# hsinnan75/Dart

Hardware: AMD Instinct MI355X
Metric: M paired-end reads/sec (2x101 bp vs GRCh38-sized index), host to host; records bit-identical to CPU dart (higher is better)
Workload: dtype u64/u8 integer

## Files before the change

### dart_amd/csrc/dg_api.hip

```cpp
#include "../../include/dartgpu.h"
#include "dg_common.h"
#include "dg_fm.h"
#include "dg_seedq.h"
#include "dg_chain.h"
#include "dg_report.h"
#include "dg_pair.h"
#include "dg_reseed.h"
#include "dg_sort.h"
#include "dg_samfmt.h"
#include "dg_bamfmt.h"
#include "dg_bgzf.h"
#include "dg_bgzf_dyn.h"
#include "dg_fastq.h"
#include "dg_inflate.h"
#include "dg_sjtab.h"
#include "dg_bamsort.h"
#include "dg_bamidx.h"
#include "dg_coverage.h"
#include "dg_markdup.h"
#include "dg_pileup.h"
#include "dg_qc.h"
#include "dg_tags.h"
#include "dg_genecount.h"
#include "dg_rnametrics.h"
#include <stdio.h>
#include <stdlib.h>
#include <string.h>
#include <string>
#include <algorithm>
#include <vector>
#include <atomic>
#include <mutex>
#include <chrono>
#include <thread>
#include <condition_variable>
#include <fcntl.h>
#include <unistd.h>
#include <sys/stat.h>

static char g_init_error[512] = "";

#define DG_HW_QUEUES_NEED 16
static_assert(DG_HW_QUEUES_NEED <= 32, "more hardware queues than 32 are not asked for");
static char g_hwq_found[24] = "unset";
static int g_hwq_left = DG_HW_QUEUES_NEED;
__attribute__((constructor)) static void dg_default_hw_queues()
{
    const char *v = getenv("GPU_MAX_HW_QUEUES");
    long have = 0;
    if (v) {
        size_t i = 0;
        for (; v[i] && i + 1 < sizeof g_hwq_found; i++) g_hwq_found[i] = (v[i] > ' ' && v[i] < 127 && v[i] != ';' && v[i] != '=') ? v[i] : '?';
        g_hwq_found[i] = 0;
        if (!i) snprintf(g_hwq_found, sizeof g_hwq_found, "empty");
        char *end = nullptr;
        have = strtol(v, &end, 10);
        if (end == v || *end) have = 0; else if (have > 1000000) have = 1000000;
    }
    if (have < DG_HW_QUEUES_NEED) {
// ... 786 lines not shown
    if (!parent) return nullptr;
    hipError_t e;
    if ((e = hipSetDevice(parent->device)) != hipSuccess) { if (status) *status = DG_ERR_HIP; return nullptr; }
    dg_ctx *c = new dg_ctx();
    c->device = parent->device; c->owns_index = false; c->n_cu = parent->n_cu;
    c->shared_ix = parent->shared_ix;
    c->ix = parent->ix; c->ix_gen = parent->ix_gen; c->pr = parent->pr;
    refresh_index(c);
    c->shared_caps = parent->shared_caps;
    if ((e = make_ctx_objects(c)) != hipSuccess) {
        snprintf(g_init_error, sizeof g_init_error, "dg_clone: %s", hipGetErrorString(e)); dg_destroy(c); if (status) *status = DG_ERR_HIP; return nullptr;
    }
    const int live = g_live_ctx[c->device & 63].load();
    if (live + 2 > g_hwq_left && !g_hwq_warned.exchange(true))
        fprintf(stderr, "[libdartgpu] %d contexts on device %d + the copy stream + the caller's stream are more than the %d hardware queues of this process "
                        "(GPU_MAX_HW_QUEUES was %s when the library loaded and %d when its constructor returned): contexts will share queues and wait for each other\n",
                live, c->device, g_hwq_left, g_hwq_found, g_hwq_left);
    if (status) *status = DG_OK;
    return c;
}

static int enqueue_upload(dg_ctx *c, int n_reads, const uint32_t *seq_off, const uint16_t *rlen, const char *seq)
{
    if (!c || n_reads < 0 || (n_reads > 0 && (!seq_off || !rlen || !seq))) return DG_ERR_ARG;
    HIPCHK(hipSetDevice(c->device));
    size_t bytes = 0; int mx = 0;
    for (int i = 0; i < n_reads; i++) {
        const size_t end = (size_t)seq_off[i] + rlen[i];
        bytes = end > bytes ? end : bytes;
        mx = rlen[i] > mx ? rlen[i] : mx;
    }
    if (mx > DG_MAX_RLEN) { snprintf(c->err, 512, "a read is longer than DG_MAX_RLEN (%d)", DG_MAX_RLEN); return DG_ERR_ARG; }
    c->n_reads = n_reads; c->max_rlen = mx; c->seq_bytes = bytes; c->enc_ready = false; c->enqueued = false; c->batch_done = false; c->sj.batch_counted = false; c->gc.batch_counted = false; c->sam.valid = false; c->bam.valid = false; c->bam.rec_valid = false; c->bam.rec_stored = false; c->fq.valid = false;
    c->no_batch = false; c->inf.valid = false;
    HIPCHK(c->seq.ensure(bytes + 64));
    HIPCHK(c->seq_off.ensure((size_t)n_reads + 1)); HIPCHK(c->rlen.ensure((size_t)n_reads + 1));
    if (n_reads) {
        HIPCHK(hipMemcpyAsync(c->seq.p, seq, bytes, hipMemcpyHostToDevice, c->stream));
        HIPCHK(hipMemcpyAsync(c->seq_off.p, seq_off, (size_t)n_reads * 4, hipMemcpyHostToDevice, c->stream));
        HIPCHK(hipMemcpyAsync(c->rlen.p, rlen, (size_t)n_reads * 2, hipMemcpyHostToDevice, c->stream));
    }
    return DG_OK;
}

extern "C" int dg_batch_upload(dg_ctx *c, int n_reads, const uint32_t *seq_off, const uint16_t *rlen, const char *seq)
{
    const int rc = enqueue_upload(c, n_reads, seq_off, rlen, seq);
    if (rc) return rc;
    HIPCHK(hipStreamSynchronize(c->stream));
    return DG_OK;
}

__global__ void __launch_bounds__(256)
k_unpack(const uint32_t *__restrict__ words, uint32_t n_words, int W2, double inv_w2, int rlen_all, const uint16_t *rlen_in, unsigned char *__restrict__ seq,
         uint32_t *__restrict__ seq_off, uint16_t *rlen_out, uint32_t *__restrict__ enc, unsigned int *bad)
{
    const uint32_t t = blockIdx.x * blockDim.x + threadIdx.x;
    if (t >= n_words) return;
    if (t == 0) *bad = 0u;
    uint32_t r = (uint32_t)((double)t * inv_w2);
    if (r * (uint32_t)W2 > t) r--; else if ((r + 1u) * (uint32_t)W2 <= t) r++;
    const int ww = (int)(t - r * (uint32_t)W2);
    const int len = rlen_in ? rlen_in[r] : rlen_all, left = len - 16 * ww;
    const uint32_t w = words[t];
    const uint32_t past = left >= 16 ? 0u : (left <= 0 ? 0xFFFFFFFFu : 0xFFFFFFFFu >> (2 * left));
    enc[(size_t)r * 2 * W2 + ww] = w & ~past;
    enc[(size_t)r * 2 * W2 + W2 + ww] = past;
    if (ww == 0) { seq_off[r] = r * 16u * (uint32_t)W2; if (!rlen_in) rlen_out[r] = (uint16_t)len; }
}
__global__ void __launch_bounds__(256)
k_unpack_n(const uint32_t *__restrict__ nlist, uint32_t n_n, int W2, uint32_t n_bases, unsigned char *__restrict__ seq, uint32_t *__restrict__ enc, unsigned int *bad)
{
    const uint32_t i = blockIdx.x * blockDim.x + threadIdx.x;
    if (i >= n_n) return;
    const uint32_t flat = nlist[i], per = 16u * (uint32_t)W2, r = flat / per, pos = flat - r * per;
    if (flat >= n_bases) { atomicMax(bad, 1u); return; }
    const uint32_t bit = 3u << (30 - 2 * (pos & 15u));
    atomicAnd(&enc[(size_t)r * 2 * W2 + (pos >> 4)], ~bit);
    atomicOr(&enc[(size_t)r * 2 * W2 + W2 + (pos >> 4)], bit);
}

static int enqueue_upload_packed(dg_ctx *c, int n_reads, int rlen_all, const uint16_t *rlen, int words_per_read, const uint32_t *words, const uint32_t *nlist, size_t n_n)
{
    if (!c || n_reads < 0 || words_per_read < 1 || (n_reads > 0 && !words) || (n_n > 0 && !nlist)) return DG_ERR_ARG;
    HIPCHK(hipSetDevice(c->device));
    const int W2 = words_per_read;
    int mx = rlen_all;
    if (rlen) { mx = 0; for (int i = 0; i < n_reads; i++) mx = rlen[i] > mx ? rlen[i] : mx; }
    if (mx > DG_MAX_RLEN || mx > 16 * W2 || (size_t)n_reads * 16 * W2 > 0xFFFFFFF0ull) { snprintf(c->err, 512, "packed batch: read length %d does not fit %d words (or exceeds DG_MAX_RLEN / 2^32 bases)", mx, W2); return DG_ERR_ARG; }
    if (n_reads && (mx + 15) / 16 != W2) { snprintf(c->err, 512, "packed batch: words_per_read must be ceil(longest read / 16) = %d", (mx + 15) / 16); return DG_ERR_ARG; }
    const size_t nw = (size_t)n_reads * W2, bytes = nw * 16;
    c->n_reads = n_reads; c->max_rlen = mx; c->seq_bytes = bytes; c->enqueued = false; c->batch_done = false; c->sj.batch_counted = false; c->gc.batch_counted = false; c->sam.valid = false; c->bam.valid = false; c->bam.rec_valid = false; c->bam.rec_stored = false; c->fq.valid = false;
    c->no_batch = false; c->inf.valid = false;
    HIPCHK(c->seq.ensure(bytes + 64)); HIPCHK(c->seq_off.ensure((size_t)n_reads + 1)); HIPCHK(c->rlen.ensure((size_t)n_reads + 1));
    HIPCHK(c->enc.ensure(2 * nw + 16)); HIPCHK(c->packed_in.ensure(nw + 1)); HIPCHK(c->nlist_in.ensure(n_n + 1));
    c->enc_ready = true;
    if (n_reads == 0) return DG_OK;
    HIPCHK(hipMemcpyAsync(c->packed_in.p, words, nw * 4, hipMemcpyHostToDevice, c->stream));
    if (rlen) HIPCHK(hipMemcpyAsync(c->rlen.p, rlen, (size_t)n_reads * 2, hipMemcpyHostToDevice, c->stream));
    if (n_n) HIPCHK(hipMemcpyAsync(c->nlist_in.p, nlist, n_n * 4, hipMemcpyHostToDevice, c->stream));
    k_unpack<<<(unsigned)((nw + 255) / 256), 256, 0, c->stream>>>(c->packed_in.p, (uint32_t)nw, W2, 1.0 / (double)W2, rlen_all, rlen ? c->rlen.p : nullptr, c->seq.p, c->seq_off.p, c->rlen.p, c->enc.p, c->d_input_bad);
    if (n_n) {
        k_unpack_n<<<(unsigned)((n_n + 255) / 256), 256, 0, c->stream>>>(c->nlist_in.p, (uint32_t)n_n, W2, (uint32_t)(nw * 16), c->seq.p, c->enc.p, c->d_input_bad);
        HIPCHK(hipMemcpyAsync(&c->h_tail->input_bad, c->d_input_bad, 4, hipMemcpyDeviceToHost, c->stream));
    } else c->h_tail->input_bad = 0;
    HIPCHK(hipGetLastError());
    return DG_OK;
}

extern "C" int dg_batch_upload_packed(dg_ctx *c, int n_reads, int rlen_all, const uint16_t *rlen, int words_per_read, const uint32_t *words, const uint32_t *nlist, size_t n_n)
{
    const int rc = enqueue_upload_packed(c, n_reads, rlen_all, rlen, words_per_read, words, nlist, n_n);
    if (rc) return rc;
    HIPCHK(hipStreamSynchronize(c->stream));
    return DG_OK;
}

extern "C" int dg_fastq_tile(void) { return FQ_TILE; }

struct FqPlan { size_t n[2], off2, line_cap[2], tile_stride, reads_bound, len_tiles, max_reads, text_bytes; bool two; };

static int fq_reserve(dg_ctx *c, FqPlan &p)
{
    HIPCHK(c->fq.ready());
    const size_t max_reads = p.max_reads, n1 = p.n[0], n2 = p.n[1];
    const size_t rec_cap[2] = { p.two ? (max_reads + 1) / 2 : max_reads, p.two ? max_reads / 2 : 0 };
    size_t tiles[2];
    for (int f = 0; f < 2; f++) { p.line_cap[f] = std::min(4 * rec_cap[f] + 1, p.n[f] + 1); tiles[f] = (p.n[f] + FQ_TILE - 1) / FQ_TILE; }
    p.off2 = (n1 + 16 + 255) & ~(size_t)255; p.text_bytes = n1 + n2;
    p.tile_stride = std::max(tiles[0], tiles[1]);
    p.reads_bound = std::min(max_reads, (n1 + 4) / 4 + (n2 + 4) / 4);
    p.len_tiles = std::max<size_t>(1, (p.reads_bound + FQ_THREADS - 1) / FQ_THREADS);
    const size_t reads_bound = p.reads_bound, text_bytes = p.text_bytes;
    HIPCHK(c->fq.text.ensure(p.off2 + n2 + 32)); HIPCHK(c->fq.lines.ensure(p.line_cap[0] + p.line_cap[1] + 2)); HIPCHK(c->fq.tile_cnt.ensure(2 * p.tile_stride + 1));
    HIPCHK(c->fq.name_at.ensure(reads_bound + 1)); HIPCHK(c->fq.name_len.ensure(reads_bound + 1)); HIPCHK(c->fq.loc.ensure(3 * (reads_bound + 1))); HIPCHK(c->fq.tile_sum.ensure(3 * p.len_tiles));
    HIPCHK(c->fq.hdr_off.ensure(reads_bound + 1)); HIPCHK(c->fq.qual_off.ensure(reads_bound + 1)); HIPCHK(c->fq.hdr.ensure(text_bytes + 1)); HIPCHK(c->fq.qual.ensure(text_bytes + 1));
    HIPCHK(c->seq.ensure(text_bytes + 64)); HIPCHK(c->seq_off.ensure(reads_bound + 1)); HIPCHK(c->rlen.ensure(reads_bound + 1));
    return DG_OK;
}

static int fq_enqueue(dg_ctx *c, const FqPlan &p, int rc_odd_reads, bool whole, bool pieces, bool write)
{
    FqText x;
    x.t[0] = c->fq.text.p; x.t[1] = c->fq.text.p + p.off2; x.n[0] = (uint32_t)p.n[0]; x.n[1] = (uint32_t)p.n[1];
    x.line_start[0] = c->fq.lines.p; x.line_start[1] = c->fq.lines.p + p.line_cap[0] + 1; x.line_cap[0] = (uint32_t)p.line_cap[0]; x.line_cap[1] = (uint32_t)p.line_cap[1];
    x.two = p.two ? 1 : 0;
    const uint32_t stride = (uint32_t)(p.reads_bound + 1);
    const dim3 text_grid((unsigned)std::max<size_t>(1, p.tile_stride), p.two ? 2u : 1u);
    k_fq_count<<<text_grid, FQ_THREADS, 0, c->stream>>>(x, c->fq.tile_cnt.p, (uint32_t)p.tile_stride);
    k_fq_top<<<1, FQ_THREADS, 0, c->stream>>>(x, c->fq.tile_cnt.p, (uint32_t)p.tile_stride, (uint32_t)p.max_reads, c->fq.info.d, whole ? 1 : 0);
    k_fq_lines<<<text_grid, FQ_THREADS, 0, c->stream>>>(x, c->fq.tile_cnt.p, (uint32_t)p.tile_stride, c->fq.info.d);
    if (whole) k_fq_tail<<<dim3(64, p.two ? 2u : 1u), FQ_THREADS, 0, c->stream>>>(x, c->fq.info.d, c->fq.tail.p, (uint32_t)c->fq.tail_off2);
    if (pieces && p.reads_bound) k_fq_unlike<<<(unsigned)p.reads_bound, 64, 0, c->stream>>>(x, c->fq.info.d);
    k_fq_len<<<(unsigned)p.len_tiles, FQ_THREADS, 0, c->stream>>>(x, c->fq.info.d, c->rlen.p, c->fq.name_at.p, c->fq.name_len.p, c->fq.loc.p, stride, c->fq.tile_sum.p, (uint32_t)p.len_tiles);
// ... 3201 lines not shown
```

### dart_amd/csrc/dg_common.h

```cpp
#pragma once
#include <hip/hip_runtime.h>
#include <stdint.h>

#define DG_WAVE 64

__host__ __device__ __forceinline__ uint64_t d_u64(uint32_t lo, uint32_t hi) { return ((uint64_t)hi << 32) | lo; }

struct __attribute__((aligned(8))) DSeed {
    int64_t  gPos;
    int32_t  rPos;
    int32_t  rLen;
    int32_t  gLen;
    uint32_t flags;
};
#define SEED_SIMPLE   1u
#define SEED_ACCEPTOR 2u

typedef uint64_t SKey;
__host__ __device__ __forceinline__ SKey sk_make(int64_t gPos, int rPos, int rLen) { return ((uint64_t)gPos << 24) | ((uint64_t)(uint32_t)rPos << 12) | (uint64_t)(uint32_t)rLen; }
__host__ __device__ __forceinline__ int64_t sk_gpos(SKey k) { return (int64_t)(k >> 24); }
__host__ __device__ __forceinline__ int sk_rpos(SKey k) { return (int)((k >> 12) & 0xFFFu); }
__host__ __device__ __forceinline__ int sk_rlen(SKey k) { return (int)(k & 0xFFFu); }
__host__ __device__ __forceinline__ int64_t sk_diag(SKey k) { return sk_gpos(k) - sk_rpos(k); }

// ... 185 lines not shown
{
    const Text64At a = d_text64_at(ix, t);
    if (!d_pac_both(ix) && a.slow) {
        uint32_t w[4] = {0u, 0u, 0u, 0u};
        for (int j = 0; j < a.nv; j++) w[j >> 4] |= (uint32_t)d_nt4((unsigned char)d_refchar(ix, t + j)) << (30 - 2 * (j & 15));
        Text64 x; x.T0 = w[0]; x.T1 = w[1]; x.T2 = w[2]; x.T3 = w[3]; x.nv = a.nv;
        return x;
    }
    const uint32_t *pw = (const uint32_t *)ix.pac + a.word;
    return d_text64_words(ix, a, pw[0], pw[1], pw[2], pw[3], pw[4]);
}

__host__ __device__ __forceinline__ void d_ref_fill(const DIndex &ix, int64_t g0, int n, char *dst)
{
    for (int i = 0; i < n; i += 8) {
        const uint64_t w = d_ref8(ix, g0 + i);
        const int m = n - i < 8 ? n - i : 8;
        for (int k = 0; k < m; k++) dst[i + k] = (char)(w >> (8 * k));
    }
}

__host__ __device__ __forceinline__ int d_loc_lower_bound(const DIndex &ix, int64_t g)
{
    int lo = 0, hi = 2 * ix.n_chr;
    while (lo < hi) { int mid = (lo + hi) >> 1; if (ix.loc_key[mid] < g) lo = mid + 1; else hi = mid; }
    return lo;
}
struct LocTab { const int64_t *key; const int32_t *chr; const int64_t *off; int n2; };
__host__ __device__ __forceinline__ LocTab d_loc_tab(const DIndex &ix) { return LocTab{ix.loc_key, ix.loc_chr, ix.chr_off, 2 * ix.n_chr}; }
__host__ __device__ __forceinline__ int d_loc_lower_bound(const LocTab &t, int64_t g)
{
    int lo = 0, hi = t.n2;
    while (lo < hi) { int mid = (lo + hi) >> 1; if (t.key[mid] < g) lo = mid + 1; else hi = mid; }
    return lo;
}

__host__ __device__ __forceinline__ bool d_seed_less(const DSeed &a, const DSeed &b)
{
    return a.gPos == b.gPos ? a.rPos < b.rPos : a.gPos < b.gPos;
}

#define CTR_STRIPES 64
#define CTR_STRIDE  48
__device__ __forceinline__ unsigned long long *d_ctr_stripe(unsigned long long *ctr) { return ctr + (blockIdx.x & (CTR_STRIPES - 1)) * CTR_STRIDE; }
__device__ __forceinline__ void d_wave_resident(unsigned long long *ctr, int which, unsigned long long t_begin)
{
    if ((threadIdx.x & 63) == 0) atomicAdd(d_ctr_stripe(ctr) + which, (unsigned long long)(wall_clock64() - t_begin));
}
__device__ __forceinline__ void d_wave_add(unsigned long long *dst, unsigned long long v)
{
    for (int o = 32; o > 0; o >>= 1) v += __shfl_down(v, o, 64);
    if ((threadIdx.x & 63) == 0 && v) atomicAdd(d_ctr_stripe(dst), v);
}
```

### dart_amd/csrc/dg_fm.h

```cpp
#pragma once
#include "dg_common.h"

struct OccBlock { uint4 q0, q1, q2, q3; };

__device__ __forceinline__ OccBlock d_load_block(const DIndex &ix, uint64_t blk)
{
    const uint4 *p = ix.bwt + (blk << 2);
    OccBlock b;
    b.q0 = p[0]; b.q1 = p[1]; b.q2 = p[2]; b.q3 = p[3];
    return b;
}

__device__ __forceinline__ uint64_t d_sel4(uint64_t a0, uint64_t a1, uint64_t a2, uint64_t a3, int i)
{
    uint64_t lo = (i & 1) ? a1 : a0, hi = (i & 1) ? a3 : a2;
    return (i & 2) ? hi : lo;
}
__device__ __forceinline__ uint64_t d_L2(const DIndex &ix, int i)
{
    return i == 4 ? ix.L2[4] : d_sel4(ix.L2[0], ix.L2[1], ix.L2[2], ix.L2[3], i);
}

__device__ __forceinline__ void d_plane_counts(const uint4 H, const uint4 Lo, uint32_t hmask, uint32_t o, uint32_t &P, uint32_t &Q)
{
// ... 634 lines not shown
                    else { h.x0 = s.x0; h.freq = (uint32_t)s.x2; }
                    hits[(size_t)r * H + at] = h;
                }
            }
            uint32_t fr = ((vh >> lane) & 1ull) ? (uint32_t)s.x2 : 0u;
            for (int o = 32; o > 0; o >>= 1) fr += (uint32_t)__shfl_xor((int)fr, o, 64);
            nh += __popcll(vh); ns += fr;
            cur += pos;
            pos = cur;
        }
        if (lane == 0) { nhits[r] = (uint32_t)nh; nseeds[r] = ns; }
    }
    d_wave_add(ctr + CTR_STEPS, c.steps);
    d_wave_add(ctr + CTR_BLOCKS, c.blocks);
    d_wave_add(ctr + CTR_STEPS_ACT, c.steps_act);
    d_wave_add(ctr + CTR_BLOCKS_ACT, c.blocks_act);
    d_wave_add(ctr + CTR_KTAB, c.ktab);
    d_wave_add(ctr + CTR_LF, c.lf_ref);
    d_wave_add(ctr + CTR_LF_ACT, c.lf_act);
    d_wave_add(ctr + CTR_DIRECT, c.n_direct);
    d_wave_resident(ctr, CTR_WT_SEEDH, t_wave0);
}

__global__ void __launch_bounds__(256)
k_build_sa_dense(const DIndex ix, int intv, uint64_t n_entries, uint64_t *__restrict__ dense)
{
    const uint64_t smask = (uint64_t)ix.sa_intv - 1, dmask = (uint64_t)intv - 1;
    const uint64_t n_sampled = (ix.seq_len + (uint64_t)ix.sa_intv) / (uint64_t)ix.sa_intv;
    int dsh = 0;
    while ((1 << dsh) < intv) dsh++;
    for (uint64_t q = (uint64_t)blockIdx.x * blockDim.x + threadIdx.x; q < n_sampled; q += (uint64_t)gridDim.x * blockDim.x) {
        const uint64_t r0 = q * (uint64_t)ix.sa_intv;
        if ((r0 >> dsh) < n_entries) dense[r0 >> dsh] = ((ix.sa[q] + 1) & 0xFFFFFFFFFFull);
        uint64_t k = d_lf(ix, r0), T = 1;
        while (k & smask) { k = d_lf(ix, k); T++; }
        const uint64_t base = ix.sa[k / (uint64_t)ix.sa_intv];
        k = d_lf(ix, r0);
        for (uint64_t t = 1; t < T; t++) {
            const uint64_t steps = T - t;
            if (!(k & dmask) && (k >> dsh) < n_entries) dense[k >> dsh] = ((steps + base + 1) & 0xFFFFFFFFFFull) | (steps << 40);
            k = d_lf(ix, k);
        }
    }
}


__global__ void __launch_bounds__(256)
k_locate(const DIndex ix, int n_reads, int H, const DHit *__restrict__ hits, const uint32_t *__restrict__ tile_read,
         const uint32_t *__restrict__ seed_off, SKey *__restrict__ seeds, unsigned long long *ctr, const int *__restrict__ abort_p)
{
    if (*abort_p >= DG_ABORT) return;
    const uint32_t total = seed_off[n_reads];
    const int lane = threadIdx.x & 63;
    const uint32_t tile = blockIdx.x * (blockDim.x >> 6) + (threadIdx.x >> 6);
    const uint32_t u = (tile << 6) + (uint32_t)lane;
    unsigned long long lf = 0, lf_act = 0, nsa = 0;
    if ((tile << 6) < total) {
        int r0 = (int)tile_read[tile];
        const uint32_t u_last = (tile << 6) + 63 < total ? (tile << 6) + 63 : total - 1;
        int r = -1;
        uint32_t first = 0;
        while (true) {
            const int rr = r0 + lane;
            const uint32_t nxt = rr + 1 <= n_reads ? seed_off[rr + 1] : 0xFFFFFFFFu;
            int lo = 0;
#pragma unroll
            for (int step = 32; step > 0; step >>= 1) {
                const uint32_t v = __shfl(nxt, lo + step - 1, 64);
                if (v <= u) lo += step;
            }
            if (__shfl(nxt, lo, 64) <= u) lo++;
            const uint32_t win_end = __shfl(nxt, 63, 64);
            if (r < 0 && u < total && lo < 64) { r = r0 + lo; first = seed_off[r]; }
            if (win_end > u_last) break;
            r0 += 64;
        }
        if (u < total) {
            uint32_t w = u - first;
            const DHit *h = hits + (size_t)r * H;
            uint32_t fr = h->freq;
            while (w >= (fr & 0x7FFFFFFFu)) { w -= fr & 0x7FFFFFFFu; h++; fr = h->freq; }
            uint64_t k = h->x0 + w;
            uint64_t steps = 0, pos;
            if (fr & 0x80000000u) pos = h->x0;
            else if (ix.sa_dense) {
                const uint64_t mask = (uint64_t)ix.sa_dense_intv - 1;
                while (k & mask) { k = d_lf(ix, k); steps++; }
                const uint64_t e = ix.sa_dense[k >> ix.sa_dense_shift];
                pos = steps + (e & 0xFFFFFFFFFFull) - 1;
                lf += steps + (e >> 40); lf_act += steps;
            } else {
                const uint64_t mask = (uint64_t)ix.sa_intv - 1;
                while (k & mask) { k = d_lf(ix, k); steps++; }
                pos = steps + ix.sa[k / (uint64_t)ix.sa_intv];
                lf += steps; lf_act += steps;
            }
            nsa++;
            seeds[u] = sk_make((int64_t)pos, (int)h->rPos, (int)h->len);
        }
    }
    d_wave_add(ctr + CTR_LF, lf);
    d_wave_add(ctr + CTR_LF_ACT, lf_act);
    d_wave_add(ctr + CTR_SA, nsa);
}
```

### dart_amd/csrc/dg_pair.h

```cpp
#pragma once
#include "../../include/dartgpu.h"
#include "dg_common.h"
#include "dg_chain.h"
#include "dg_report.h"

template <class R1, class R2>
__host__ __device__ inline void d_settle_pair(const DParams &pr, DRead &m1, R1 &p1, DRead &m2, R2 &p2)
{
    bool linked = p1.mate(m1.iBest) == m2.iBest;
    if (linked && !pr.multi_hit) return;
    if (!linked && m1.score > 0 && m2.score > 0) {
        int best_sum = 0;
        for (int i = 0; i < m1.CanNum; i++) {
            const int a = p1.aln(i), j = p1.mate(i);
            if (a <= 0 || j < 0) continue;
            const int b = p2.aln(j);
            if (b <= 0) continue;
            linked = true;
            if (a + b > best_sum) { best_sum = a + b; m1.iBest = i; m1.score = a; m2.iBest = j; m2.score = b; }
        }
    }
    if (linked) {
        for (int i = 0; i < m1.CanNum; i++) {
            const int j = p1.mate(i);
// ... 435 lines not shown
    const unsigned long long pp_t0 = st.pt;
#endif
    int r1 = 0, n1 = 0, n2 = 0, len1 = 0, len2 = 0;
    uint32_t b1 = 0;
    uint32_t pf = 0, pf2 = 0, pf3 = 0, pf4 = 0, pf5 = 0, pf6 = 0;
    bool heavy = false;
    if (valid) {
        r1 = paired ? 2 * u : u;
        len1 = rlen[r1]; len2 = paired ? rlen[r1 + 1] : 0;
        if (PACKED) { pf = enc[(size_t)r1 * 2 * W2 + (W2 >> 1)]; if (paired) pf2 = enc[(size_t)(r1 + 1) * 2 * W2 + (W2 >> 1)]; }
        b1 = seed_off[r1];
        const uint32_t e1 = seed_off[r1 + 1], e2 = paired ? seed_off[r1 + 2] : e1;
        n1 = (int)(e1 - b1); n2 = (int)(e2 - e1);
        heavy = n1 + n2 > PU_SEEDS;
        if (!heavy) {
            const SKey *src = seeds + b1;
            const int nt = n1 + n2;
            for (int i0 = 0; i0 < nt; i0 += 4) {
                const SKey k0 = src[i0], k1 = i0 + 1 < nt ? src[i0 + 1] : 0, k2 = i0 + 2 < nt ? src[i0 + 2] : 0, k3 = i0 + 3 < nt ? src[i0 + 3] : 0;
                key[i0 * PU_THREADS] = k0;
                if (i0 + 1 < nt) key[(i0 + 1) * PU_THREADS] = k1;
                if (i0 + 2 < nt) key[(i0 + 2) * PU_THREADS] = k2;
                if (i0 + 3 < nt) key[(i0 + 3) * PU_THREADS] = k3;
            }
#ifdef __HIP_DEVICE_COMPILE__
            __asm__ volatile("" ::: "memory");
#endif
            if (n1 > 1) { pf3 = d_pac_touch(ix, key[0]); if (n1 > 2) pf4 = d_pac_touch(ix, key[1 * PU_THREADS]); }
            if (n2 > 1) { pf5 = d_pac_touch(ix, key[n1 * PU_THREADS]); if (n2 > 2) pf6 = d_pac_touch(ix, key[(n1 + 1) * PU_THREADS]); }
            PP_STAMP(st.pp, st.pt, 0);
            if (PACKED) {
                const ReadWords a{enc + (size_t)r1 * 2 * W2, W2}, b{enc + (size_t)(r1 + (paired ? 1 : 0)) * 2 * W2, W2};
                d_unit_process_rd<PU_THREADS, ReadWords>(ix, lt, pr, paired != 0, n1, n2, len1, len2, a, b, key, cw, rw, try_fast != 0, st);
            } else d_unit_process_rd<PU_THREADS, ReadAscii>(ix, lt, pr, paired != 0, n1, n2, len1, len2, ReadAscii{seq + seq_off[r1]}, ReadAscii{seq + seq_off[r1 + (paired ? 1 : 0)]}, key, cw, rw, try_fast != 0, st);
        } else { st.nc[0] = (int)ncand[r1]; st.nc[1] = paired ? (int)ncand[r1 + 1] : 0; }
    }
    const uint32_t nrep1 = valid ? (uint32_t)(st.nc[0] > 0 ? st.nc[0] : 1) : 0u, nrep2 = (valid && paired) ? (uint32_t)(st.nc[1] > 0 ? st.nc[1] : 1) : 0u;
    Triple mine, tot;
    mine.x = nrep1 + nrep2; mine.y = (valid && !st.fast) ? 1u : 0u; mine.z = st.fast ? st.n_cig : 0u;
    uint32_t cc1 = 0;
    mine.w = 0;
    if (co.reads && st.fast) {
        RepLds<PU_THREADS> q1{cw, rw, st.nc[0], st.flag0[0]}, q2{cw + st.nc[0] * PU_THREADS, rw, st.nc[1], st.flag0[1]};
        cc1 = d_unit_compact_ops<PU_THREADS>(st.rd[0], q1);
        mine.w = cc1 + (paired ? d_unit_compact_ops<PU_THREADS>(st.rd[1], q2) : 0u);
    }
    PP_STAMP(st.pp, st.pt, 5);
    const Triple inb = d_block_exclusive(mine, tot, s_scan);
    PP_STAMP(st.pp, st.pt, 6);
    const Triple base = d_tile_exclusive(ts, tile, tot, s_scan + 16, err);
    PP_STAMP(st.pp, st.pt, 7);
    const uint32_t rep0 = base.x + inb.x, slow_at = base.y + inb.y;
    const uint64_t cig0 = base.z + inb.z;
    unsigned long long n_cands = 0, n_nw = 0, n_cells = 0;
    if (valid) {
        rep_off[r1] = rep0;
        if (paired) rep_off[r1 + 1] = rep0 + nrep1;
        if (!heavy) n_cands = (unsigned long long)(st.nc[0] + st.nc[1]);
        if (st.fast) {
            if ((uint64_t)rep0 + mine.x > cap_rep) atomicMax(err, DG_E_REPORTS);
            else if (cig0 + st.n_cig > cap_cig) atomicMax(err, DG_E_CIGFINAL);
            else {
                RepLds<PU_THREADS> p1{cw, rw, st.nc[0], st.flag0[0]}, p2{cw + st.nc[0] * PU_THREADS, rw, st.nc[1], st.flag0[1]};
                const uint32_t cigc0 = base.w + inb.w;
                const bool full = !(write_all_sorted & 2) || !co.reads;
                const uint32_t c1 = d_unit_emit_read<PU_THREADS>(true, st.rd[0], p1, rep0, (uint32_t)cig0, rout + r1, reports, cigar, co, co.reads ? co.reads + r1 : nullptr, cigc0, full);
                if (paired) d_unit_emit_read<PU_THREADS>(false, st.rd[1], p2, rep0 + nrep1, (uint32_t)cig0 + c1, rout + r1 + 1, reports, cigar, co, co.reads ? co.reads + r1 + 1 : nullptr, cigc0 + cc1, full);
                n_nw = st.n_nw; n_cells = st.n_cells;
            }
        } else {
            if (slow_at < (uint32_t)n_units) slow_units[slow_at] = (uint32_t)u;
            if ((uint64_t)rep0 + mine.x > cap_rep) atomicMax(err, DG_E_REPORTS);
        }
        if (!heavy && (!st.fast || (write_all_sorted & 1))) {
            const int nt = n1 + n2;
            for (int i = 0; i < nt; i++) seeds[b1 + i] = key[i * PU_THREADS];
            auto put_cands = [&](int first_cw, int first_key, uint32_t seg, int count, int r) {
                for (int i = 0; i < count; i++) {
                    const uint32_t w = cw[(first_cw + i) * PU_THREADS];
                    const int64_t d = sk_diag(key[(first_key + cw_first(w)) * PU_THREADS]);
                    DCand c = d_new_cand(seg + (uint32_t)cw_first(w), cw_count(w), cw_score(w), d < 0 ? 0 : d);
                    c.PairedIdx = cw_mate(w);
                    cands[seg + i] = c;
                }
                ncand[r] = (uint32_t)count;
            };
            put_cands(0, 0, b1, st.nc[0], r1);
            if (paired) put_cands(st.nc[0], n1, b1 + (uint32_t)n1, st.nc[1], r1 + 1);
        } else if (!heavy) { ncand[r1] = (uint32_t)st.nc[0]; if (paired) ncand[r1 + 1] = (uint32_t)st.nc[1]; }
    }
    if (tile == gridDim.x - 1 && threadIdx.x == 0) {
        sizes->total_rep = base.x + tot.x; sizes->n_slow_units = base.y + tot.y; sizes->cig_fast = (uint32_t)(base.z + tot.z);
        sizes->total_cig = sizes->cig_fast;
        sizes->pad[2] = base.w + tot.w;
        *pool_top = (base.x + tot.x) * CIG_SLOT;
    }
    PP_STAMP(st.pp, st.pt, 8);
#ifdef DG_PAIR_PROF
    if ((threadIdx.x & 63) == 0 && (tile % 61u) == 0u)
        printf("kpair tile %u wave %d: total %llu | load %llu sort+cluster %llu rules %llu reports %llu settle %llu rest %llu blockscan %llu lookback %llu emit %llu\n", tile, (int)(threadIdx.x >> 6),
               __builtin_amdgcn_s_memtime() - pp_t0, st.pp[0], st.pp[1], st.pp[2], st.pp[3], st.pp[4], st.pp[5], st.pp[6], st.pp[7], st.pp[8]);
#endif
    if (n_units < 0 && (pf ^ pf2 ^ pf3 ^ pf4 ^ pf5 ^ pf6) == 0x5A17C3E1u) atomicMax(err, DG_E_SCAN);
    d_wave_add(ctr + CTR_CANDS, n_cands);
    d_wave_add(ctr + CTR_NW, n_nw);
    d_wave_add(ctr + CTR_NWCELLS, n_cells);
    d_wave_resident(ctr, CTR_WT_PAIR, t_wave0);
}
```

Baseline: 1216.

## Restructure unpack per 64-read wave, add full-SA fast path, cheaper wave counters

Replaces the per-word unpack kernel with a per-wave kernel in which each wave handles 64 reads, using a magic-multiply division instead of a double-precision reciprocal. The SA-lookup kernel gains a fast path for a fully dense suffix array that skips LF walks, loads hits as uint4, and uses readlane/readfirstlane for uniform values. Wave-level counter reductions switch to 32-bit DPP sums or ballot popcounts in the SA and pair kernels to cut shuffle cost. A standalone probe compares the unpack variants. These are small kernels and counters, so the end-to-end effect is likely minor.

```diff
diff --git a/dart_amd/csrc/dg_api.hip b/dart_amd/csrc/dg_api.hip
--- a/dart_amd/csrc/dg_api.hip
+++ b/dart_amd/csrc/dg_api.hip
@@ -5,6 +5,7 @@
 #include "dg_chain.h"
 #include "dg_report.h"
 #include "dg_pair.h"
+#include "dg_unpack.h"
 #include "dg_reseed.h"
 #include "dg_sort.h"
 #include "dg_samfmt.h"
@@ -897,23 +898,6 @@
 }
 
 __global__ void __launch_bounds__(256)
-k_unpack(const uint32_t *__restrict__ words, uint32_t n_words, int W2, double inv_w2, int rlen_all, const uint16_t *rlen_in, unsigned char *__restrict__ seq,
-         uint32_t *__restrict__ seq_off, uint16_t *rlen_out, uint32_t *__restrict__ enc, unsigned int *bad)
-{
-    const uint32_t t = blockIdx.x * blockDim.x + threadIdx.x;
-    if (t >= n_words) return;
-    if (t == 0) *bad = 0u;
-    uint32_t r = (uint32_t)((double)t * inv_w2);
-    if (r * (uint32_t)W2 > t) r--; else if ((r + 1u) * (uint32_t)W2 <= t) r++;
-    const int ww = (int)(t - r * (uint32_t)W2);
-    const int len = rlen_in ? rlen_in[r] : rlen_all, left = len - 16 * ww;
-    const uint32_t w = words[t];
-    const uint32_t past = left >= 16 ? 0u : (left <= 0 ? 0xFFFFFFFFu : 0xFFFFFFFFu >> (2 * left));
-    enc[(size_t)r * 2 * W2 + ww] = w & ~past;
-    enc[(size_t)r * 2 * W2 + W2 + ww] = past;
-    if (ww == 0) { seq_off[r] = r * 16u * (uint32_t)W2; if (!rlen_in) rlen_out[r] = (uint16_t)len; }
-}
-__global__ void __launch_bounds__(256)
 k_unpack_n(const uint32_t *__restrict__ nlist, uint32_t n_n, int W2, uint32_t n_bases, unsigned char *__restrict__ seq, uint32_t *__restrict__ enc, unsigned int *bad)
 {
     const uint32_t i = blockIdx.x * blockDim.x + threadIdx.x;
@@ -944,7 +928,7 @@
     HIPCHK(hipMemcpyAsync(c->packed_in.p, words, nw * 4, hipMemcpyHostToDevice, c->stream));
     if (rlen) HIPCHK(hipMemcpyAsync(c->rlen.p, rlen, (size_t)n_reads * 2, hipMemcpyHostToDevice, c->stream));
     if (n_n) HIPCHK(hipMemcpyAsync(c->nlist_in.p, nlist, n_n * 4, hipMemcpyHostToDevice, c->stream));
-    k_unpack<<<(unsigned)((nw + 255) / 256), 256, 0, c->stream>>>(c->packed_in.p, (uint32_t)nw, W2, 1.0 / (double)W2, rlen_all, rlen ? c->rlen.p : nullptr, c->seq.p, c->seq_off.p, c->rlen.p, c->enc.p, c->d_input_bad);
+    k_unpack<<<(unsigned)(((size_t)n_reads + 255) / 256), 256, 0, c->stream>>>(c->packed_in.p, (uint32_t)n_reads, W2, d_unpack_magic(W2), rlen_all, rlen ? c->rlen.p : nullptr, c->seq_off.p, c->rlen.p, c->enc.p, c->d_input_bad);
     if (n_n) {
         k_unpack_n<<<(unsigned)((n_n + 255) / 256), 256, 0, c->stream>>>(c->nlist_in.p, (uint32_t)n_n, W2, (uint32_t)(nw * 16), c->seq.p, c->enc.p, c->d_input_bad);
         HIPCHK(hipMemcpyAsync(&c->h_tail->input_bad, c->d_input_bad, 4, hipMemcpyDeviceToHost, c->stream));
diff --git a/dart_amd/csrc/dg_common.h b/dart_amd/csrc/dg_common.h
--- a/dart_amd/csrc/dg_common.h
+++ b/dart_amd/csrc/dg_common.h
@@ -261,3 +261,18 @@
     for (int o = 32; o > 0; o >>= 1) v += __shfl_down(v, o, 64);
     if ((threadIdx.x & 63) == 0 && v) atomicAdd(d_ctr_stripe(dst), v);
 }
+__device__ __forceinline__ void d_wave_add32(unsigned long long *dst, uint32_t v)
+{
+    v += (uint32_t)__builtin_amdgcn_update_dpp(0, (int)v, 0x111, 0xF, 0xF, false);
+    v += (uint32_t)__builtin_amdgcn_update_dpp(0, (int)v, 0x112, 0xF, 0xF, false);
+    v += (uint32_t)__builtin_amdgcn_update_dpp(0, (int)v, 0x114, 0xF, 0xF, false);
+    v += (uint32_t)__builtin_amdgcn_update_dpp(0, (int)v, 0x118, 0xF, 0xF, false);
+    v += (uint32_t)__builtin_amdgcn_update_dpp(0, (int)v, 0x142, 0xA, 0xF, false);
+    v += (uint32_t)__builtin_amdgcn_update_dpp(0, (int)v, 0x143, 0xC, 0xF, false);
+    if ((threadIdx.x & 63) == 63 && v) atomicAdd(d_ctr_stripe(dst), (unsigned long long)v);
+}
+__device__ __forceinline__ void d_wave_add_lanes(unsigned long long *dst, bool mine)
+{
+    const unsigned long long b = __ballot(mine);
+    if ((threadIdx.x & 63) == 0 && b) atomicAdd(d_ctr_stripe(dst), (unsigned long long)__popcll(b));
+}
diff --git a/dart_amd/csrc/dg_fm.h b/dart_amd/csrc/dg_fm.h
--- a/dart_amd/csrc/dg_fm.h
+++ b/dart_amd/csrc/dg_fm.h
@@ -710,54 +710,61 @@
     if (*abort_p >= DG_ABORT) return;
     const uint32_t total = seed_off[n_reads];
     const int lane = threadIdx.x & 63;
-    const uint32_t tile = blockIdx.x * (blockDim.x >> 6) + (threadIdx.x >> 6);
-    const uint32_t u = (tile << 6) + (uint32_t)lane;
-    unsigned long long lf = 0, lf_act = 0, nsa = 0;
-    if ((tile << 6) < total) {
-        int r0 = (int)tile_read[tile];
-        const uint32_t u_last = (tile << 6) + 63 < total ? (tile << 6) + 63 : total - 1;
-        int r = -1;
-        uint32_t first = 0;
-        while (true) {
-            const int rr = r0 + lane;
-            const uint32_t nxt = rr + 1 <= n_reads ? seed_off[rr + 1] : 0xFFFFFFFFu;
-            int lo = 0;
+    const uint32_t tile = blockIdx.x * (blockDim.x >> 6) + (uint32_t)__builtin_amdgcn_readfirstlane((int)(threadIdx.x >> 6));
+    const uint32_t u0 = tile << 6, u = u0 + (uint32_t)lane;
+    if (u0 >= total) return;
+    const bool act = u < total;
+    int r0 = (int)tile_read[tile];
+    const uint32_t u_last = u0 + 63 < total ? u0 + 63 : total - 1;
+    int r = -1;
+    uint32_t first = 0;
+    while (true) {
+        const int rr = r0 + lane;
+        const uint32_t nxt = rr + 1 <= n_reads ? seed_off[rr + 1] : 0xFFFFFFFFu;
+        int lo = 0;
 #pragma unroll
-            for (int step = 32; step > 0; step >>= 1) {
-                const uint32_t v = __shfl(nxt, lo + step - 1, 64);
-                if (v <= u) lo += step;
-            }
-            if (__shfl(nxt, lo, 64) <= u) lo++;
-            const uint32_t win_end = __shfl(nxt, 63, 64);
-            if (r < 0 && u < total && lo < 64) { r = r0 + lo; first = seed_off[r]; }
-            if (win_end > u_last) break;
-            r0 += 64;
-        }
-        if (u < total) {
-            uint32_t w = u - first;
-            const DHit *h = hits + (size_t)r * H;
-            uint32_t fr = h->freq;
-            while (w >= (fr & 0x7FFFFFFFu)) { w -= fr & 0x7FFFFFFFu; h++; fr = h->freq; }
-            uint64_t k = h->x0 + w;
-            uint64_t steps = 0, pos;
-            if (fr & 0x80000000u) pos = h->x0;
-            else if (ix.sa_dense) {
-                const uint64_t mask = (uint64_t)ix.sa_dense_intv - 1;
-                while (k & mask) { k = d_lf(ix, k); steps++; }
-                const uint64_t e = ix.sa_dense[k >> ix.sa_dense_shift];
-                pos = steps + (e & 0xFFFFFFFFFFull) - 1;
-                lf += steps + (e >> 40); lf_act += steps;
-            } else {
-                const uint64_t mask = (uint64_t)ix.sa_intv - 1;
-                while (k & mask) { k = d_lf(ix, k); steps++; }
-                pos = steps + ix.sa[k / (uint64_t)ix.sa_intv];
-                lf += steps; lf_act += steps;
-            }
-            nsa++;
-            seeds[u] = sk_make((int64_t)pos, (int)h->rPos, (int)h->len);
-        }
-    }
-    d_wave_add(ctr + CTR_LF, lf);
-    d_wave_add(ctr + CTR_LF_ACT, lf_act);
-    d_wave_add(ctr + CTR_SA, nsa);
-}
+        for (int step = 32; step > 0; step >>= 1) {
+            const uint32_t v = __shfl(nxt, lo + step - 1, 64);
+            if (v <= u) lo += step;
+        }
+        if (__shfl(nxt, lo, 64) <= u) lo++;
+        const uint32_t win_end = (uint32_t)__builtin_amdgcn_readlane((int)nxt, 63);
+        if (r < 0 && act && lo < 64) { r = r0 + lo; first = seed_off[r]; }
+        if (win_end > u_last) break;
+        r0 += 64;
+    }
+    const bool full_sa = ix.sa_dense != nullptr && ix.sa_dense_intv == 1;
+    uint32_t lf32 = 0;
+    unsigned long long lf = 0, lf_act = 0;
+    if (act) {
+        uint32_t w = u - first;
+        const uint4 *hp = (const uint4 *)(hits + (size_t)r * H);
+        uint4 h = *hp;
+        while (w >= (h.z & 0x7FFFFFFFu)) { w -= h.z & 0x7FFFFFFFu; h = *++hp; }
+        const uint64_t x0 = d_u64(h.x, h.y);
+        uint64_t pos;
+        if (h.z & 0x80000000u) pos = x0;
+        else if (full_sa) {
+            const uint64_t e = ix.sa_dense[x0 + w];
+            pos = (e & 0xFFFFFFFFFFull) - 1;
+            lf32 = (uint32_t)(e >> 40);
+        } else if (ix.sa_dense) {
+            const uint64_t mask = (uint64_t)ix.sa_dense_intv - 1;
+            uint64_t k = x0 + w, steps = 0;
+            while (k & mask) { k = d_lf(ix, k); steps++; }
+            const uint64_t e = ix.sa_dense[k >> ix.sa_dense_shift];
+            pos = steps + (e & 0xFFFFFFFFFFull) - 1;
+            lf = steps + (e >> 40); lf_act = steps;
+        } else {
+            const uint64_t mask = (uint64_t)ix.sa_intv - 1;
+            uint64_t k = x0 + w, steps = 0;
+            while (k & mask) { k = d_lf(ix, k); steps++; }
+            pos = steps + ix.sa[k / (uint64_t)ix.sa_intv];
+            lf = lf_act = steps;
+        }
+        seeds[u] = sk_make((int64_t)pos, (int)(h.w & 0xFFFFu), (int)(h.w >> 16));
+    }
+    if (full_sa) d_wave_add32(ctr + CTR_LF, lf32);
+    else { d_wave_add(ctr + CTR_LF, lf); d_wave_add(ctr + CTR_LF_ACT, lf_act); }
+    d_wave_add_lanes(ctr + CTR_SA, act);
+}
diff --git a/dart_amd/csrc/dg_pair.h b/dart_amd/csrc/dg_pair.h
--- a/dart_amd/csrc/dg_pair.h
+++ b/dart_amd/csrc/dg_pair.h
@@ -511,11 +511,11 @@
     PP_STAMP(st.pp, st.pt, 7);
     const uint32_t rep0 = base.x + inb.x, slow_at = base.y + inb.y;
     const uint64_t cig0 = base.z + inb.z;
-    unsigned long long n_cands = 0, n_nw = 0, n_cells = 0;
+    uint32_t n_cands = 0, n_nw = 0, n_cells = 0;
     if (valid) {
         rep_off[r1] = rep0;
         if (paired) rep_off[r1 + 1] = rep0 + nrep1;
-        if (!heavy) n_cands = (unsigned long long)(st.nc[0] + st.nc[1]);
+        if (!heavy) n_cands = (uint32_t)(st.nc[0] + st.nc[1]);
         if (st.fast) {
             if ((uint64_t)rep0 + mine.x > cap_rep) atomicMax(err, DG_E_REPORTS);
             else if (cig0 + st.n_cig > cap_cig) atomicMax(err, DG_E_CIGFINAL);
@@ -561,8 +561,9 @@
                __builtin_amdgcn_s_memtime() - pp_t0, st.pp[0], st.pp[1], st.pp[2], st.pp[3], st.pp[4], st.pp[5], st.pp[6], st.pp[7], st.pp[8]);
 #endif
     if (n_units < 0 && (pf ^ pf2 ^ pf3 ^ pf4 ^ pf5 ^ pf6) == 0x5A17C3E1u) atomicMax(err, DG_E_SCAN);
-    d_wave_add(ctr + CTR_CANDS, n_cands);
-    d_wave_add(ctr + CTR_NW, n_nw);
-    d_wave_add(ctr + CTR_NWCELLS, n_cells);
+    static_assert(PU_SEEDS <= 32 && SMALL_NW <= 8, "the bounds of k_pair's 32-bit wave sums");
+    d_wave_add32(ctr + CTR_CANDS, n_cands);
+    d_wave_add32(ctr + CTR_NW, n_nw);
+    d_wave_add32(ctr + CTR_NWCELLS, n_cells);
     d_wave_resident(ctr, CTR_WT_PAIR, t_wave0);
 }
diff --git a/dart_amd/csrc/dg_unpack.h b/dart_amd/csrc/dg_unpack.h
--- /dev/null
+++ b/dart_amd/csrc/dg_unpack.h
@@ -0,0 +1,68 @@
+#pragma once
+#include "../../include/dartgpu.h"
+#include "dg_common.h"
+
+__host__ __device__ __forceinline__ uint32_t d_unpack_past(int left)
+{
+    const int l = left < 0 ? 0 : (left > 16 ? 16 : left);
+    return (uint32_t)(0xFFFFFFFFull >> (2 * l));
+}
+
+#define UNPACK_SHIFT 18
+__host__ __device__ __forceinline__ uint32_t d_unpack_magic(int W2) { return (1u << UNPACK_SHIFT) / (uint32_t)W2 + 1u; }
+static_assert((DG_MAX_RLEN + 15) / 16 <= 63, "d_unpack_magic: a tile of 64 reads holds at most 64 * 63 words");
+
+template <bool FULL, bool PER_READ>
+__host__ __device__ __forceinline__ void d_unpack_tile(int lane, uint32_t r0, int nrd, int W2, uint32_t magic, int rlen_all, const uint16_t *rlen_in,
+                                                       const uint32_t *__restrict__ words, uint32_t *__restrict__ enc, uint32_t *__restrict__ seq_off, uint16_t *rlen_out)
+{
+    const char *in = (const char *)(words + (size_t)r0 * (uint32_t)W2);
+    char *out = (char *)(enc + (size_t)r0 * 2u * (uint32_t)W2);
+    const char *len_of = PER_READ ? (const char *)(rlen_in + r0) : nullptr;
+    const uint32_t nw = (uint32_t)nrd * (uint32_t)W2, row = 4u * (uint32_t)W2;
+    uint32_t i = (uint32_t)lane;
+    for (int j = 0; j < W2; j++, i += 64u) {
+        if (!FULL && i >= nw) break;
+        const uint32_t ro = (i * magic) >> UNPACK_SHIFT;
+#ifdef __HIP_DEVICE_COMPILE__
+        const uint32_t t = __umul24(ro, (uint32_t)W2);
+#else
+        const uint32_t t = ro * (uint32_t)W2;
+#endif
+        const int len = PER_READ ? (int)*(const uint16_t *)(len_of + (ro << 1)) : rlen_all;
+        const uint32_t past = d_unpack_past(len + (int)(t - i) * 16), o = (i + t) << 2;
+        *(uint32_t *)(out + o) = *(const uint32_t *)(in + (i << 2)) & ~past;
+        *(uint32_t *)(out + (o + row)) = past;
+    }
+    if (FULL || lane < nrd) {
+        const uint32_t r = r0 + (uint32_t)lane;
+        seq_off[r] = r * 16u * (uint32_t)W2;
+        if (!PER_READ) rlen_out[r] = (uint16_t)rlen_all;
+    }
+}
+
+__host__ __device__ __forceinline__ void d_unpack_wave(uint32_t tile, int lane, const uint32_t *__restrict__ words, uint32_t n_reads, int W2, uint32_t magic, int rlen_all,
+                                                       const uint16_t *rlen_in, uint32_t *__restrict__ seq_off, uint16_t *rlen_out, uint32_t *__restrict__ enc, unsigned int *bad)
+{
+    const uint32_t r0 = tile << 6;
+    if (r0 >= n_reads) return;
+    if (tile == 0 && lane == 0) *bad = 0u;
+    const int nrd = n_reads - r0 >= 64u ? 64 : (int)(n_reads - r0);
+    if (rlen_in) {
+        if (nrd == 64) d_unpack_tile<true, true>(lane, r0, 64, W2, magic, rlen_all, rlen_in, words, enc, seq_off, rlen_out);
+        else d_unpack_tile<false, true>(lane, r0, nrd, W2, magic, rlen_all, rlen_in, words, enc, seq_off, rlen_out);
+    } else {
+        if (nrd == 64) d_unpack_tile<true, false>(lane, r0, 64, W2, magic, rlen_all, rlen_in, words, enc, seq_off, rlen_out);
+        else d_unpack_tile<false, false>(lane, r0, nrd, W2, magic, rlen_all, rlen_in, words, enc, seq_off, rlen_out);
+    }
+}
+
+__global__ void __launch_bounds__(256)
+k_unpack(const uint32_t *__restrict__ words, uint32_t n_reads, int W2, uint32_t magic, int rlen_all, const uint16_t *rlen_in,
+         uint32_t *__restrict__ seq_off, uint16_t *rlen_out, uint32_t *__restrict__ enc, unsigned int *bad)
+{
+#ifdef __HIP_DEVICE_COMPILE__
+    const uint32_t tile = blockIdx.x * (blockDim.x >> 6) + (uint32_t)__builtin_amdgcn_readfirstlane((int)(threadIdx.x >> 6));
+    d_unpack_wave(tile, (int)(threadIdx.x & 63u), words, n_reads, W2, magic, rlen_all, rlen_in, seq_off, rlen_out, enc, bad);
+#endif
+}
diff --git a/profiles/probes/unpack_probe.hip b/profiles/probes/unpack_probe.hip
--- /dev/null
+++ b/profiles/probes/unpack_probe.hip
@@ -0,0 +1,87 @@
+#include "../../dart_amd/csrc/dg_unpack.h"
+#include <stdio.h>
+#include <stdlib.h>
+#include <algorithm>
+#include <vector>
+
+#define CHK(x) do { hipError_t e_ = (x); if (e_ != hipSuccess) { fprintf(stderr, "%s:%d %s\n", __FILE__, __LINE__, hipGetErrorString(e_)); return 1; } } while (0)
+
+__global__ void __launch_bounds__(256)
+k_unpack_word(const uint32_t *__restrict__ words, uint32_t n_words, int W2, double inv_w2, int rlen_all, const uint16_t *rlen_in,
+              uint32_t *__restrict__ seq_off, uint16_t *rlen_out, uint32_t *__restrict__ enc, unsigned int *bad)
+{
+    const uint32_t t = blockIdx.x * blockDim.x + threadIdx.x;
+    if (t >= n_words) return;
+    if (t == 0) *bad = 0u;
+    uint32_t r = (uint32_t)((double)t * inv_w2);
+    if (r * (uint32_t)W2 > t) r--; else if ((r + 1u) * (uint32_t)W2 <= t) r++;
+    const int ww = (int)(t - r * (uint32_t)W2);
+    const int len = rlen_in ? rlen_in[r] : rlen_all, left = len - 16 * ww;
+    const uint32_t w = words[t];
+    const uint32_t past = left >= 16 ? 0u : (left <= 0 ? 0xFFFFFFFFu : 0xFFFFFFFFu >> (2 * left));
+    enc[(size_t)r * 2 * W2 + ww] = w & ~past;
+    enc[(size_t)r * 2 * W2 + W2 + ww] = past;
+    if (ww == 0) { seq_off[r] = r * 16u * (uint32_t)W2; if (!rlen_in) rlen_out[r] = (uint16_t)len; }
+}
+
+__global__ void __launch_bounds__(256)
+k_unpack_lane(const uint32_t *__restrict__ words, uint32_t n_reads, int W2, int rlen_all, const uint16_t *rlen_in,
+              uint32_t *__restrict__ seq_off, uint16_t *rlen_out, uint32_t *__restrict__ enc, unsigned int *bad)
+{
+    const uint32_t r = blockIdx.x * blockDim.x + threadIdx.x;
+    if (r >= n_reads) return;
+    if (r == 0) *bad = 0u;
+    const int len = rlen_in ? rlen_in[r] : rlen_all;
+    const uint32_t *in = words + (size_t)r * W2;
+    uint32_t *out = enc + (size_t)r * 2 * W2;
+    for (int ww = 0; ww < W2; ww++) {
+        const uint32_t past = d_unpack_past(len - 16 * ww);
+        out[ww] = in[ww] & ~past;
+        out[W2 + ww] = past;
+    }
+    seq_off[r] = r * 16u * (uint32_t)W2;
+    if (!rlen_in) rlen_out[r] = (uint16_t)len;
+}
+
+int main(int argc, char **argv)
+{
+    const uint32_t n = argc > 1 ? (uint32_t)atoll(argv[1]) : 2000000u;
+    const int rlen = argc > 2 ? atoi(argv[2]) : 101, reps = argc > 3 ? atoi(argv[3]) : 20;
+    const int W2 = (rlen + 15) / 16;
+    if (n == 0 || rlen < 1 || rlen > DG_MAX_RLEN || (size_t)n * 16 * W2 > 0xFFFFFFF0ull || reps < 1) { fprintf(stderr, "bad arguments\n"); return 2; }
+    const size_t nw = (size_t)n * W2;
+    std::vector<uint32_t> h(nw);
+    uint64_t s = 88172645463325252ull;
+    for (auto &w : h) { s ^= s << 13; s ^= s >> 7; s ^= s << 17; w = (uint32_t)(s >> 16); }
+    uint32_t *words, *enc[3], *seq_off; uint16_t *rl; unsigned int *bad;
+    CHK(hipMalloc(&words, (nw + 1) * 4)); CHK(hipMalloc(&seq_off, ((size_t)n + 1) * 4)); CHK(hipMalloc(&rl, ((size_t)n + 1) * 2)); CHK(hipMalloc(&bad, 4));
+    for (int v = 0; v < 3; v++) { CHK(hipMalloc(&enc[v], (2 * nw + 16) * 4)); CHK(hipMemset(enc[v], 0x5A, (2 * nw + 16) * 4)); }
+    CHK(hipMemcpy(words, h.data(), nw * 4, hipMemcpyHostToDevice));
+    hipEvent_t e0, e1;
+    CHK(hipEventCreate(&e0)); CHK(hipEventCreate(&e1));
+    const char *name[3] = {"thread = word (before)", "wave = 64 reads (k_unpack)", "thread = read"};
+    for (int v = 0; v < 3; v++) {
+        std::vector<float> ms;
+        for (int k = 0; k < reps + 2; k++) {
+            CHK(hipEventRecord(e0, 0));
+            if (v == 0) k_unpack_word<<<(unsigned)((nw + 255) / 256), 256>>>(words, (uint32_t)nw, W2, 1.0 / (double)W2, rlen, nullptr, seq_off, rl, enc[0], bad);
+            if (v == 1) k_unpack<<<(unsigned)(((size_t)n + 255) / 256), 256>>>(words, n, W2, d_unpack_magic(W2), rlen, nullptr, seq_off, rl, enc[1], bad);
+            if (v == 2) k_unpack_lane<<<(unsigned)(((size_t)n + 255) / 256), 256>>>(words, n, W2, rlen, nullptr, seq_off, rl, enc[2], bad);
+            CHK(hipEventRecord(e1, 0)); CHK(hipEventSynchronize(e1)); CHK(hipGetLastError());
+            float t; CHK(hipEventElapsedTime(&t, e0, e1));
+            if (k >= 2) ms.push_back(t);
+        }
+        std::sort(ms.begin(), ms.end());
+        printf("%-28s reads %u rlen %d: median %.4f ms, min %.4f, max %.4f over %d launches (%.0f GB/s of %zu MB moved)\n", name[v], n, rlen, ms[ms.size() / 2], ms.front(), ms.back(), reps,
+               12.0 * nw / ms[ms.size() / 2] / 1e6, 12 * nw >> 20);
+    }
+    std::vector<uint32_t> a(2 * nw), b(2 * nw);
+    CHK(hipMemcpy(a.data(), enc[0], 2 * nw * 4, hipMemcpyDeviceToHost));
+    int differ = 0;
+    for (int v = 1; v < 3; v++) {
+        CHK(hipMemcpy(b.data(), enc[v], 2 * nw * 4, hipMemcpyDeviceToHost));
+        differ += a != b;
+    }
+    printf("outputs %s\n", differ ? "DIFFER" : "identical");
+    return differ;
+}
```

Measured after the change: 1182. 2.8% lower.
